# cshizhe/VLN-HAMT

Measured on AMD Instinct MI355X. Metric: panorama-steps/sec, R2R proxy pretrain (36x768 views, 80-tok instr), higher is better.
Workload: dtype bf16; 1 GPU; R2R 6-proxy-task pretrain step (fwd+bwd+clip+AdamW, dropout 0.1), fixed ViT features, R2R-canon model 174.8M params; per_gpu_batch=64, global_batch=64, txt_len=80, hist_len=5, views=36, task_mix=mlm:sap:sar:sprel:mrc:itm=5:1:1:1:2:2, parallelism=dp1, launch=hipGraph replay, dead_code_elimination=True

## Files before the change

### include/hamt.h

```cpp
#ifndef HAMT_H
#define HAMT_H

#include <stddef.h>
#include <stdint.h>

#ifdef __cplusplus
extern "C" {
#endif

#define HAMT_ABI_VERSION 2

typedef enum { HAMT_OK = 0, HAMT_ERR_ARG = -1, HAMT_ERR_UNSUPPORTED = -2, HAMT_ERR_LAUNCH = -3 } hamt_status;
typedef enum { HAMT_F32 = 0, HAMT_BF16 = 1,
               HAMT_U8G = 2,
               HAMT_F16 = 3 } hamt_dtype;
typedef enum { HAMT_PREC_BF16 = 0, HAMT_PREC_F32 = 1 } hamt_prec;

int hamt_version(void);
int hamt_last_error(char* buf, size_t n);
int hamt_last_kernel(char* buf, size_t n);
enum { HAMT_WS_GEMM_SPLITK = 0, HAMT_WS_COLSUM = 1, HAMT_WS_SUMSQ = 2, HAMT_WS_LN_BWD = 3, HAMT_WS_WGRAD_TABLE = 4, HAMT_WS_LNRED_TABLE = 5, HAMT_WS_VIS_EMBED_BWD = 6,
       HAMT_WS_EMBED_BWD = 7 ,
       HAMT_WS_OBJ_EMBED_BWD = 8, HAMT_WS_IMAGE_PREP = 9  };
size_t hamt_workspace_bytes(int op, const int* shape, int nshape);
// ... 37 lines not shown
  const void* dy;
  const void* x;
  float* dw;
  float* db;
  int M, N, K, ldy, ldx, ldw;
  int accum_dw, accum_db;
  float* ss;
  int K_valid;
  float wire_scale;
  const void* dy2;
  const void* x2;
  int K2, ldy2, ldx2, K2_valid;
} hamt_wgrad_desc;
#define HAMT_WGRAD_TABLE_ENTRY 112
int hamt_wgrad_grouped(int n, const hamt_wgrad_desc* probs, void* table, size_t table_bytes, void* stream);
int hamt_wgrad_grouped_ex(int n, const hamt_wgrad_desc* probs, void* table, size_t table_bytes, int phase, void* stream);

int hamt_colsum(int M, int N, const void* x, int ldx, int dtype_x, float* out, int accumulate,
                float* ws, void* stream);

typedef struct {
  int B, heads, Sq, Sk, d_head;
  int ldq, ldk, ldv, ldo;
  int dtype_qkv, dtype_o;
  float scale, p_drop;
  uint32_t call_id;
  int prec;
} hamt_attn_desc;
int hamt_attn_small_fwd(const hamt_attn_desc* d, const void* q, const void* k, const void* v,
                        const float* add_mask, void* o, float* lse, const uint64_t* rng, void* stream);
int hamt_attn_small_bwd(const hamt_attn_desc* d, const void* q, const void* k, const void* v,
                        const float* add_mask, const void* o, const void* d_o, const float* lse,
                        float* delta, void* dq, void* dk, void* dv, const uint64_t* rng, void* stream);

int hamt_attn_cls_fwd(const hamt_attn_desc* d, const void* q, const void* k, const void* v, void* o, void* stream);

int hamt_attn_varlen_fwd(const hamt_attn_desc* d, const void* q, const void* k, const void* v, const int* cu_seqlens,
                         void* o, float* lse, const uint64_t* rng, void* stream);
int hamt_attn_varlen_bwd(const hamt_attn_desc* d, const void* q, const void* k, const void* v, const int* cu_seqlens,
                         const void* o, const void* d_o, const float* lse, void* dq, void* dk, void* dv,
                         const uint64_t* rng, void* stream);
int hamt_attn_varlen_cross_fwd(const hamt_attn_desc* d, const void* q, const void* k, const void* v, const int* cu_q,
                               const int* cu_k, int n_pairs, const int* pair, const float* add_mask, void* o, float* lse,
                               const uint64_t* rng, void* stream);
int hamt_attn_varlen_cross_bwd(const hamt_attn_desc* d, const void* q, const void* k, const void* v, const int* cu_q,
                               const int* cu_k, int n_pairs, const int* pair, const float* add_mask, const void* o, const void* d_o,
                               const float* lse, void* dq, void* dk, void* dv, const uint64_t* rng, void* stream);

typedef struct {
  int M, H;
  int A;
  int ld_ang;
  float eps1, eps2;
  int x_bf16;
  int Mpad16;
} hamt_vis_embed_desc;
int hamt_vis_embed_fwd(const hamt_vis_embed_desc* d, const void* x1, const float* ang, const float* w_ang, const float* b_ang,
                       const float* gamma_img, const float* beta_img, const float* gamma_ang, const float* beta_ang,
                       float* y, void* y16, float* stats, void* stream);
int hamt_vis_embed_bwd(const hamt_vis_embed_desc* d, const float* dy, const void* x1, const float* ang, const float* w_ang,
                       const float* b_ang, const float* gamma_img, const float* gamma_ang, const float* stats, float* dx, void* dx16,
                       float* dgamma_img, float* dbeta_img, float* dgamma_ang, float* dbeta_ang, float* db_ang, float* dw_ang,
                       float* ws, void* stream);

typedef struct {
  int M, H;
// ... 280 lines not shown
```

### vln_hamt_amd/_lib.py

```python
from __future__ import annotations

import ctypes as C
import os

_HERE = os.path.dirname(os.path.abspath(__file__))
LIB_PATH = os.path.join(_HERE, "libhamt_hip.so")

HAMT_F32, HAMT_BF16, HAMT_U8G, HAMT_F16 = 0, 1, 2, 3
PREC_BF16, PREC_F32 = 0, 1
EPI_BIAS, EPI_GELU, EPI_RELU, EPI_ACCUM, EPI_MUL_DGELU, EPI_MUL_DRELU, EPI_SAVE_PRE = 1, 2, 4, 8, 16, 32, 64
EPI_GELU_GRAD, EPI_MUL_AUX, EPI_ADD_AUX, EPI_DROPOUT = 128, 256, 512, 1024
SUMSQ_SPARSE = 2
OPT_ADAMW, OPT_ADAM, OPT_RMSPROP, OPT_SGD = 0, 1, 2, 3

vp, i32, u32, f32, sz = C.c_void_p, C.c_int, C.c_uint32, C.c_float, C.c_size_t


class GemmDesc(C.Structure):
    _fields_ = [("M", i32), ("N", i32), ("K", i32), ("lda", i32), ("ldb", i32), ("ldc", i32), ("ldaux", i32),
                ("a_kmajor", i32), ("b_kmajor", i32), ("dtype_a", i32), ("dtype_b", i32), ("dtype_c", i32),
                ("dtype_aux", i32), ("prec", i32), ("epilogue", i32), ("alpha", f32), ("ka_rows", i32), ("kb_rows", i32),
                ("p_drop", f32), ("call_id", u32), ("rng", C.c_void_p)]


# ... 56 lines not shown


class ImageResampleDesc(C.Structure):
    _fields_ = [(n, i32) for n in ("n", "H", "W", "OH", "OW", "x0", "y0", "w", "h", "filter", "kx", "ky")]


WGRAD_TABLE_ENTRY = 112


class WgradDesc(C.Structure):
    _fields_ = [("dy", vp), ("x", vp), ("dw", vp), ("db", vp), ("M", i32), ("N", i32), ("K", i32), ("ldy", i32),
                ("ldx", i32), ("ldw", i32), ("accum_dw", i32), ("accum_db", i32), ("ss", vp), ("K_valid", i32),
                ("wire_scale", f32), ("dy2", vp), ("x2", vp), ("K2", i32), ("ldy2", i32), ("ldx2", i32), ("K2_valid", i32)]


SIGNATURES = {
    "hamt_version": [],
    "hamt_last_error": [C.c_char_p, sz],
    "hamt_last_kernel": [C.c_char_p, sz],
    "hamt_workspace_bytes": [i32, C.POINTER(i32), i32],
    "hamt_gemm": [C.POINTER(GemmDesc), vp, vp, vp, vp, vp, vp],
    "hamt_gemm_ksplit": [C.POINTER(GemmDesc)],
    "hamt_gemm_ws": [C.POINTER(GemmDesc), vp, vp, vp, vp, vp, vp, sz, vp],
    "hamt_gemm_plan": [C.POINTER(GemmDesc), sz, C.c_char_p, sz],
    "hamt_cast_pad_bf16": [i32, i32, i32, i32, vp, i32, vp, i32, vp],
    "hamt_cast_pad_bf16_dropout": [i32, i32, i32, vp, i32, vp, i32, f32, u32, vp, vp],
    "hamt_cast_transpose": [i32, i32, vp, i32, i32, vp, i32, i32, vp],
    "hamt_wgrad_grouped": [i32, C.POINTER(WgradDesc), vp, sz, vp],
    "hamt_wgrad_grouped_ex": [i32, C.POINTER(WgradDesc), vp, sz, i32, vp],
    "hamt_smallk_wgrad": [i32, i32, i32, vp, i32, vp, i32, vp, i32, vp, vp],
    "hamt_colsum": [i32, i32, vp, i32, i32, vp, i32, vp, vp],
    "hamt_attn_small_fwd": [C.POINTER(AttnDesc), vp, vp, vp, vp, vp, vp, vp, vp],
    "hamt_attn_small_bwd": [C.POINTER(AttnDesc), vp, vp, vp, vp, vp, vp, vp, vp, vp, vp, vp, vp, vp],
    "hamt_attn_cls_fwd": [C.POINTER(AttnDesc), vp, vp, vp, vp, vp],
    "hamt_attn_varlen_fwd": [C.POINTER(AttnDesc), vp, vp, vp, vp, vp, vp, vp, vp],
    "hamt_attn_varlen_bwd": [C.POINTER(AttnDesc), vp, vp, vp, vp, vp, vp, vp, vp, vp, vp, vp, vp],
    "hamt_attn_varlen_cross_fwd": [C.POINTER(AttnDesc), vp, vp, vp, vp, vp, C.c_int, vp, vp, vp, vp, vp, vp],
    "hamt_attn_varlen_cross_bwd": [C.POINTER(AttnDesc), vp, vp, vp, vp, vp, C.c_int, vp, vp, vp, vp, vp, vp, vp, vp, vp, vp],
    "hamt_vis_embed_fwd": [C.POINTER(VisEmbedDesc)] + [vp] * 12,
    "hamt_vis_embed_bwd": [C.POINTER(VisEmbedDesc)] + [vp] * 18,
    "hamt_obj_embed_fwd": [C.POINTER(ObjEmbedDesc), C.POINTER(ObjEmbedParams)] + [vp] * 7,
    "hamt_obj_embed_bwd": [C.POINTER(ObjEmbedDesc), C.POINTER(ObjEmbedParams), C.POINTER(ObjEmbedGrads)] + [vp] * 10,
    "hamt_ln_fwd": [C.POINTER(LnDesc), vp, vp, vp, vp, vp, vp, vp, vp, vp, vp, vp],
    "hamt_ln_bwd": [C.POINTER(LnDesc), vp, vp, vp, vp, vp, vp, vp, vp, vp, vp, vp, vp, vp, vp],
    "hamt_ln_bwd_add": [C.POINTER(LnDesc), vp, vp, vp, vp, vp, vp, vp, vp, vp, vp, vp],
    "hamt_ln_bwd_reduce": [i32, i32, vp, vp, vp, vp, vp],
    "hamt_ln_bwd_reduce_grouped": [i32, vp, vp, sz, vp],
    "hamt_gather_rows": [i32, i32, vp, i32, vp, vp, i32, vp, i32, i32, vp],
    "hamt_scatter_add_rows": [i32, i32, vp, i32, i32, vp, vp, i32, vp],
    "hamt_scatter_add_rows_small": [i32, i32, vp, i32, i32, vp, i32, vp, vp, vp],
    "hamt_scatter_add_rows_ordered": [i32, i32, vp, i32, i32, vp, vp, i32, i32, vp, vp],
    "hamt_embed_sum_fwd": [i32, i32, i32, vp, vp, vp, vp, vp, vp],
    "hamt_embed_sum_bwd": [i32, i32, i32, i32, vp, vp, vp, vp, vp, vp, sz, vp],
    "hamt_mean_mid_fwd": [i32, i32, i32, vp, vp, vp],
    "hamt_mean_mid_bwd": [i32, i32, i32, vp, vp, vp],
    "hamt_mul_bcast_fwd": [i32, i32, i32, vp, vp, i32, vp, vp],
    "hamt_mul_bcast_bwd": [i32, i32, i32, vp, vp, i32, vp, vp, vp, vp],
    "hamt_sum_rows": [i32, i32, i32, vp, i32, vp, vp, vp],
    "hamt_patchify": [i32, i32, i32, i32, i32, vp, vp, i32, i32, i32, vp],
    "hamt_image_prep": [C.POINTER(ImagePrepDesc), vp, vp, vp, vp, vp, vp, sz, vp],
    "hamt_image_resample_taps": [i32, i32, i32, i32, i32, vp, vp, vp, i32],
    "hamt_image_resample": [C.POINTER(ImageResampleDesc), vp, vp, vp, vp, vp, vp, vp],
    "hamt_add3": [sz, vp, vp, vp, vp, vp],
    "hamt_dropout": [sz, vp, vp, f32, u32, vp, vp],
    "hamt_cast_f32_bf16": [sz, vp, vp, vp],
    "hamt_unpack_padded": [vp, vp, i32, i32, i32, i32, vp, vp],
# ... 65 lines not shown
        raise HamtError(f"{LIB_PATH} is missing: build it with `python vln_hamt_amd/csrc/build.py` "
                        "(there is no CPU/PyTorch fallback for the HAMT kernels)")
    import torch
    lib = C.CDLL(LIB_PATH)
    for name, args in SIGNATURES.items():
        fn = getattr(lib, name)
        fn.argtypes = args
        fn.restype = sz if name == "hamt_workspace_bytes" else i32
    if lib.hamt_version() != 2:
        raise HamtError("libhamt_hip.so ABI version mismatch")
    _lib = lib
    return lib


def last_error() -> str:
    buf = C.create_string_buffer(512)
    load().hamt_last_error(buf, 512)
    return buf.value.decode(errors="replace")


def last_kernel() -> str:
    buf = C.create_string_buffer(160)
    load().hamt_last_kernel(buf, 160)
    return buf.value.decode(errors="replace")


def gemm_plan(desc: GemmDesc, ws_bytes=None):
    buf = C.create_string_buffer(160)
    ks = load().hamt_gemm_plan(C.byref(desc), sz(-1).value if ws_bytes is None else ws_bytes, buf, 160)
    check(min(ks, 0), "hamt_gemm_plan")
    return ks, buf.value.decode(errors="replace")


def workspace_bytes(op: int, *shape) -> int:
    arr = (i32 * max(1, len(shape)))(*shape)
    return int(load().hamt_workspace_bytes(op, arr, len(shape)))


WS_GEMM_SPLITK, WS_COLSUM, WS_SUMSQ, WS_LN_BWD, WS_WGRAD_TABLE, WS_LNRED_TABLE, WS_VIS_EMBED_BWD, WS_EMBED_BWD, WS_OBJ_EMBED_BWD = range(9)
WS_IMAGE_PREP = 9


def check(rc: int, name: str):
    if rc != 0:
        raise HamtError(f"{name} failed (status {rc}): {last_error()}")
```

### vln_hamt_amd/csrc/attn16.hip

```cpp
#include "common.h"

namespace {

constexpr int T64 = 64;
constexpr int AST = 72;
typedef __attribute__((address_space(3))) s16x4 lds_s16x4;

struct Attn16Args {
  hamt_attn_desc d;
  const void *q, *k, *v, *o, *d_o;
  const float* mask;
  void *out, *dq, *dk, *dv;
  float* lse;
  const uint64_t* rng;
  const int* cu_q;
  const int* cu_k;
  int n_pairs;
  const int* pair;
};

template <typename T> __device__ __forceinline__ void ld8(const T* p, float (&f)[8]);
template <> __device__ __forceinline__ void ld8<float>(const float* p, float (&f)[8]) {
  const float4 a = ((const float4*)p)[0], b = ((const float4*)p)[1];
  f[0] = a.x; f[1] = a.y; f[2] = a.z; f[3] = a.w; f[4] = b.x; f[5] = b.y; f[6] = b.z; f[7] = b.w;
}
template <> __device__ __forceinline__ void ld8<bf16_t>(const bf16_t* p, float (&f)[8]) {
  const uint4 x = *(const uint4*)p;
  const uint32_t u[4] = {x.x, x.y, x.z, x.w};
#pragma unroll
  for (int j = 0; j < 4; ++j) { f[2 * j] = __uint_as_float(u[j] << 16); f[2 * j + 1] = __uint_as_float(u[j] & 0xffff0000u); }
}
__device__ __forceinline__ uint4 pack8(const float (&f)[8]) {
  return make_uint4(pack_bf2(f[0], f[1]), pack_bf2(f[2], f[3]), pack_bf2(f[4], f[5]), pack_bf2(f[6], f[7]));
}
template <typename T> __device__ __forceinline__ void st4(T* p, float a, float b, float c, float d);
template <> __device__ __forceinline__ void st4<float>(float* p, float a, float b, float c, float d) { *(float4*)p = make_float4(a, b, c, d); }
template <> __device__ __forceinline__ void st4<bf16_t>(bf16_t* p, float a, float b, float c, float d) { *(uint2*)p = make_uint2(pack_bf2(a, b), pack_bf2(c, d)); }
template <typename T> __device__ __forceinline__ float4 ld4(const T* p);
// ... 419 lines not shown
  float rs = 0.f;
  f32x4 of[4];
#pragma unroll
  for (int i = 0; i < 4; ++i) of[i] = (f32x4){0.f, 0.f, 0.f, 0.f};
#pragma unroll
  for (int s = 0; s < KB / 2; ++s) {
    float p[2][4];
#pragma unroll
    for (int e = 0; e < 2; ++e) {
#pragma unroll
      for (int r = 0; r < 4; ++r) { p[e][r] = __expf(sf[2 * s + e][r] - mn); rs += p[e][r]; }
      if (d.p_drop > 0.f) {
        float ds4[4];
        drop_scale4(key, rowh, (uint32_t)(4 * (2 * s + e) + g), d.p_drop, inv_keep, ds4);
#pragma unroll
        for (int r = 0; r < 4; ++r) p[e][r] *= ds4[r];
      }
    }
    const bf16x8 pf = pack_frag(p[0], p[1]);
#pragma unroll
    for (int db = 0; db < 4; ++db) of[db] = MFMA16(tfrag(Vs, 32 * s + 4 * g, 32 * s + 16 + 4 * g, 16 * db, lane), pf, of[db]);
  }
  const float l_run = xg_sum(rs);
  if (qok) {
    TO* O = (TO*)a.out + qrow0 * d.ldo + h * 64 + (size_t)qrow * d.ldo;
    const float inv = 1.0f / l_run;
#pragma unroll
    for (int db = 0; db < 4; ++db) st4<TO>(O + 16 * db + 4 * g, of[db][0] * inv, of[db][1] * inv, of[db][2] * inv, of[db][3] * inv);
    if (g == 0) a.lse[((size_t)b * d.heads + h) * d.Sq + qrow] = mn + __logf(l_run);
  }
}

template <typename TI, typename TO, int NB>
__global__ __launch_bounds__(512) void attn_s128_bwd_kernel(Attn16Args a) {
  extern __shared__ __attribute__((aligned(16))) bf16_t sm[];
  const hamt_attn_desc& d = a.d;
  const int t = threadIdx.x, nt = blockDim.x, lane = t & 63, w = t >> 6, l15 = lane & 15, g = lane >> 4;
  const int h = blockIdx.x, b = blockIdx.y;
  int Sq = d.Sq, Sk = d.Sk;
  size_t qrow0 = (size_t)b * d.Sq, krow0 = (size_t)b * d.Sk;
  if (a.cu_q) { const int c0 = a.cu_q[b]; Sq = a.cu_q[b + 1] - c0; qrow0 = (size_t)c0; }
  if (Sq <= 0) return;
  const int kb_ = a.pair ? a.pair[b] : b;
  const bool filler = a.pair ? kb_ < 0 : ((a.cu_q || a.cu_k) && b >= a.n_pairs);
  if (!filler) {
    krow0 = (size_t)kb_ * d.Sk;
    if (a.cu_k) { const int c0 = a.cu_k[kb_]; Sk = a.cu_k[kb_ + 1] - c0; krow0 = (size_t)c0; }
  }
  if (filler || Sk <= 0) {
    TI* dQ0 = (TI*)a.dq + qrow0 * d.ldq + h * 64;
    for (int i = t; i < Sq * 8; i += nt) { st4<TI>(dQ0 + (size_t)(i >> 3) * d.ldq + (i & 7) * 8, 0.f, 0.f, 0.f, 0.f); st4<TI>(dQ0 + (size_t)(i >> 3) * d.ldq + (i & 7) * 8 + 4, 0.f, 0.f, 0.f, 0.f); }
    return;
  }
  const int nqb = (Sq + 15) >> 4, nkb = (Sk + 15) >> 4, sq16 = nqb * 16, sk16 = nkb * 16, PST = sq16 + 8;
  bf16_t* Qs = sm;
  bf16_t* dOs = Qs + sq16 * AST;
  bf16_t* Ks = dOs + sq16 * AST;
  bf16_t* Vs = Ks + sk16 * AST;
  bf16_t* Pt = Vs + sk16 * AST;
  bf16_t* dSt = Pt + sk16 * PST;
  float* lse_s = (float*)(dSt + sk16 * PST);
  float* delta_s = lse_s + sq16;
  float* mk_s = delta_s + sq16;
  const TI* Q = (const TI*)a.q + qrow0 * d.ldq + h * 64;
  const TI* K = (const TI*)a.k + krow0 * d.ldk + h * 64;
  const TI* V = (const TI*)a.v + krow0 * d.ldv + h * 64;
  const TO* O = (const TO*)a.o + qrow0 * d.ldo + h * 64;
  const TO* dO = (const TO*)a.d_o + qrow0 * d.ldo + h * 64;
  {
    Raw8<TI> rq[2], rk[2], rv[2];
    Raw8<TO> rdo[2], ro[2];
    rows_load<TI, 2>(Q, d.ldq, Sq, t, nt, rq);
    rows_load<TO, 2>(dO, d.ldo, Sq, t, nt, rdo);
    rows_load<TO, 2>(O, d.ldo, Sq, t, nt, ro);
    rows_load<TI, 2>(K, d.ldk, Sk, t, nt, rk);
    rows_load<TI, 2>(V, d.ldv, Sk, t, nt, rv);
    stage_mask(a.cu_k ? nullptr : a.mask, kb_, Sk, sk16, mk_s, t, nt);
    for (int i = t; i < sk16 * PST / 8; i += nt) { ((uint4*)Pt)[i] = make_uint4(0, 0, 0, 0); ((uint4*)dSt)[i] = make_uint4(0, 0, 0, 0); }
    rows_store<TI, 2>(rq, sq16, Qs, t, nt);
    rows_store<TO, 2>(rdo, sq16, dOs, t, nt);
#pragma unroll
    for (int i = 0; i < 2; ++i) {
      const int r = (t >> 3) + i * (nt >> 3);
      float f[8], o8[8], acc = 0.f;
      raw_f32(rdo[i], f);
      raw_f32(ro[i], o8);
#pragma unroll
      for (int j = 0; j < 8; ++j) acc += f[j] * o8[j];
      acc += __shfl_xor(acc, 1, 64); acc += __shfl_xor(acc, 2, 64); acc += __shfl_xor(acc, 4, 64);
      if ((t & 7) == 0 && r < sq16) { delta_s[r] = acc; lse_s[r] = r < Sq ? a.lse[((size_t)b * d.heads + h) * d.Sq + r] : 0.f; }
    }
    rows_store<TI, 2>(rk, sk16, Ks, t, nt);
    rows_store<TI, 2>(rv, sk16, Vs, t, nt);
  }
  __syncthreads();
  const RngKey key = rng_key(a.rng, d.call_id);
  const float inv_keep = d.p_drop > 0.f ? 1.0f / (1.0f - d.p_drop) : 1.0f;
  if (w < nqb) {
    const int ql = 16 * w + l15;
    bf16x8 qf[2], df[2];
#pragma unroll
    for (int s = 0; s < 2; ++s) { qf[s] = rfrag(Qs, ql, 32 * s + 8 * g); df[s] = rfrag(dOs, ql, 32 * s + 8 * g); }
    const float lse_q = lse_s[ql], delta_q = delta_s[ql];
    const uint32_t rowh = hamt_mix32((uint32_t)((b * d.heads + h) * d.Sq + ql) ^ key.k0);
    const bool qv = ql < Sq;
#pragma unroll
    for (int kb = 0; kb < NB; ++kb) {
      if (kb < nkb) {
        f32x4 sf = (f32x4){0.f, 0.f, 0.f, 0.f}, dpf = (f32x4){0.f, 0.f, 0.f, 0.f};
#pragma unroll
        for (int s = 0; s < 2; ++s) {
          sf = MFMA16(rfrag(Ks, 16 * kb + l15, 32 * s + 8 * g), qf[s], sf);
          dpf = MFMA16(rfrag(Vs, 16 * kb + l15, 32 * s + 8 * g), df[s], dpf);
        }
        const float4 mk = *(const float4*)(mk_s + 16 * kb + 4 * g);
        const float mk4[4] = {mk.x, mk.y, mk.z, mk.w};
        float ds4[4] = {1.f, 1.f, 1.f, 1.f};
        if (d.p_drop > 0.f) drop_scale4(key, rowh, (uint32_t)(4 * kb + g), d.p_drop, inv_keep, ds4);
#pragma unroll
        for (int r = 0; r < 4; ++r) {
          const int kk = 16 * kb + 4 * g + r;
          const float pr = __expf(fmaf(sf[r], d.scale, mk4[r]) - lse_q);
          if (qv) {
            Pt[kk * PST + ql] = f2bf(pr * ds4[r]);
            dSt[kk * PST + ql] = f2bf(pr * (dpf[r] * ds4[r] - delta_q) * d.scale);
          }
        }
      }
    }
  }
  __syncthreads();
  if (w < nkb) {
    f32x4 dkf[4], dvf[4];
#pragma unroll
    for (int i = 0; i < 4; ++i) { dkf[i] = (f32x4){0.f, 0.f, 0.f, 0.f}; dvf[i] = (f32x4){0.f, 0.f, 0.f, 0.f}; }
#pragma unroll
    for (int s = 0; s < NB / 2; ++s) {
      if (2 * s < nqb) {
        const bf16x8 pb = rfrag_lim(Pt, PST, 16 * w + l15, 32 * s + 8 * g, sq16), sb = rfrag_lim(dSt, PST, 16 * w + l15, 32 * s + 8 * g, sq16);
#pragma unroll
        for (int db = 0; db < 4; ++db) {
          dvf[db] = MFMA16(tfrag_lim(dOs, AST, 32 * s + 8 * g, 32 * s + 8 * g + 4, sq16, 16 * db, lane), pb, dvf[db]);
          dkf[db] = MFMA16(tfrag_lim(Qs, AST, 32 * s + 8 * g, 32 * s + 8 * g + 4, sq16, 16 * db, lane), sb, dkf[db]);
        }
      }
    }
    const int kk = 16 * w + l15;
    if (kk < Sk) {
      TI* dK = (TI*)a.dk + krow0 * d.ldk + h * 64 + (size_t)kk * d.ldk;
      TI* dV = (TI*)a.dv + krow0 * d.ldv + h * 64 + (size_t)kk * d.ldv;
#pragma unroll
      for (int db = 0; db < 4; ++db) {
        st4<TI>(dK + 16 * db + 4 * g, dkf[db][0], dkf[db][1], dkf[db][2], dkf[db][3]);
        st4<TI>(dV + 16 * db + 4 * g, dvf[db][0], dvf[db][1], dvf[db][2], dvf[db][3]);
      }
    }
  }
  if (w < nqb) {
    f32x4 dqf[4];
#pragma unroll
    for (int i = 0; i < 4; ++i) dqf[i] = (f32x4){0.f, 0.f, 0.f, 0.f};
#pragma unroll
    for (int s = 0; s < NB / 2; ++s) {
      if (2 * s < nkb) {
        const bf16x8 sb = tfrag_lim(dSt, PST, 32 * s + 8 * g, 32 * s + 8 * g + 4, sk16, 16 * w, lane);
#pragma unroll
        for (int db = 0; db < 4; ++db) dqf[db] = MFMA16(tfrag_lim(Ks, AST, 32 * s + 8 * g, 32 * s + 8 * g + 4, sk16, 16 * db, lane), sb, dqf[db]);
      }
    }
    const int qq = 16 * w + l15;
    if (qq < Sq) {
      TI* dQ = (TI*)a.dq + qrow0 * d.ldq + h * 64 + (size_t)qq * d.ldq;
#pragma unroll
      for (int db = 0; db < 4; ++db) st4<TI>(dQ + 16 * db + 4 * g, dqf[db][0], dqf[db][1], dqf[db][2], dqf[db][3]);
    }
  }
}

template <typename TI, typename TO, bool PACKED>
__global__ __launch_bounds__(1024) void attn_wide_bwd_kernel(Attn16Args a) {
  extern __shared__ __attribute__((aligned(16))) bf16_t sm[];
  const hamt_attn_desc& d = a.d;
  const int t = threadIdx.x, nt = blockDim.x, lane = t & 63, w = t >> 6, l15 = lane & 15, g = lane >> 4;
  const int h = blockIdx.x, b = blockIdx.y;
  int Sq = d.Sq, Sk = d.Sk;
  size_t qrow0 = (size_t)b * d.Sq, krow0 = (size_t)b * d.Sk;
  const float* mask = a.mask;
  int mrow = b;
  if constexpr (PACKED) {
    if (a.cu_q) { const int c0 = a.cu_q[b]; Sq = a.cu_q[b + 1] - c0; qrow0 = (size_t)c0; }
    if (Sq <= 0) return;
    mrow = a.pair ? a.pair[b] : b;
    const bool filler = a.pair ? mrow < 0 : b >= a.n_pairs;
    if (!filler) {
      krow0 = (size_t)mrow * d.Sk;
      if (a.cu_k) { const int c0 = a.cu_k[mrow]; Sk = a.cu_k[mrow + 1] - c0; krow0 = (size_t)c0; mask = nullptr; }
    }
    if (filler || Sk <= 0) {
      TI* dQ0 = (TI*)a.dq + qrow0 * d.ldq + h * 64;
      for (int i = t; i < Sq * 16; i += nt) st4<TI>(dQ0 + (size_t)(i >> 4) * d.ldq + (i & 15) * 4, 0.f, 0.f, 0.f, 0.f);
      return;
    }
  }
  const int nqb = (Sq + 15) >> 4, nkb = (Sk + 15) >> 4, sq16 = nqb * 16, sk16 = nkb * 16;
  bf16_t* Qs = sm;
// ... 119 lines not shown
          for (int r = 0; r < 4; ++r) {
            const float pr = __expf(fmaf(sf[r], d.scale, mk) - lq[r]);
            float keep = 1.f;
            if (d.p_drop > 0.f) {
              uint32_t x = hamt_mix32(rh[r] + grp_h);
              if (second) x = hamt_mix32(x ^ 0x85ebca6bu);
              keep = (high ? (x >> 16) : (x & 0xffffu)) >= thr ? inv_keep : 0.0f;
            }
            const bool qv = 16 * qb + 4 * g + r < Sq;
            pt[e][r] = qv ? pr * keep : 0.f;
            dsv[e][r] = qv ? pr * (dpf[r] * keep - dq_[r]) * d.scale : 0.f;
          }
        }
      }
      const bf16x8 pb = pack_frag(pt[0], pt[1]), sb = pack_frag(dsv[0], dsv[1]);
#pragma unroll
      for (int db = 0; db < 4; ++db) {
        dvf[db] = MFMA16(tfrag_lim(dOs, AST, 32 * s + 4 * g, 32 * s + 16 + 4 * g, sq16, 16 * db, lane), pb, dvf[db]);
        dkf[db] = MFMA16(tfrag_lim(Qs, AST, 32 * s + 4 * g, 32 * s + 16 + 4 * g, sq16, 16 * db, lane), sb, dkf[db]);
      }
    }
    if (kl < Sk) {
      TI* dK = (TI*)a.dk + krow0 * d.ldk + h * 64 + (size_t)kl * d.ldk;
      TI* dV = (TI*)a.dv + krow0 * d.ldv + h * 64 + (size_t)kl * d.ldv;
#pragma unroll
      for (int db = 0; db < 4; ++db) {
        st4<TI>(dK + 16 * db + 4 * g, dkf[db][0], dkf[db][1], dkf[db][2], dkf[db][3]);
        st4<TI>(dV + 16 * db + 4 * g, dvf[db][0], dvf[db][1], dvf[db][2], dvf[db][3]);
      }
    }
  }
}

size_t wide_bwd_lds(const hamt_attn_desc& d) {
  const int sq16 = (d.Sq + 15) / 16 * 16, sk16 = (d.Sk + 15) / 16 * 16;
  return (size_t)2 * (sq16 + sk16) * AST * sizeof(bf16_t) + (size_t)(3 * sq16 + sk16) * sizeof(float);
}

template <typename TI, typename TO, bool PACKED>
void launch_wide_bwd(const Attn16Args& a, hipStream_t s) {
  const hamt_attn_desc& d = a.d;
  const int nqb = (d.Sq + 15) / 16, nkb = (d.Sk + 15) / 16, nb = nqb > nkb ? nqb : nkb;
  static bool raised = false;
  if (!raised) {
    (void)hipFuncSetAttribute(reinterpret_cast<const void*>(&attn_wide_bwd_kernel<TI, TO, PACKED>), hipFuncAttributeMaxDynamicSharedMemorySize, 160 * 1024);
    raised = true;
  }
  hipLaunchKernelGGL((attn_wide_bwd_kernel<TI, TO, PACKED>), dim3(d.heads, d.B), dim3(64 * nb), wide_bwd_lds(d), s, a);
}

template <typename TI, typename TO, int KB, int IT>
void launch_s128_fwd_kb(const Attn16Args& a, dim3 grid, dim3 block, size_t lds, hipStream_t s) {
  static bool raised = false;
  if (lds > 64 * 1024 && !raised) {
    hipFuncSetAttribute(reinterpret_cast<const void*>(&attn_s128_fwd_kernel<TI, TO, KB, IT>), hipFuncAttributeMaxDynamicSharedMemorySize, 160 * 1024);
    raised = true;
  }
  hipLaunchKernelGGL((attn_s128_fwd_kernel<TI, TO, KB, IT>), grid, block, lds, s, a);
}

template <typename TI, typename TO>
void launch_s128_fwd(const Attn16Args& a, hipStream_t s) {
  const hamt_attn_desc& d = a.d;
  const int nqb = (d.Sq + 15) / 16, nkb = (d.Sk + 15) / 16;
  const int kb = nkb <= 2 ? 2 : (nkb + 1) & ~1;
  const int it = kb > 8 ? 4 : 2;
  const int need = 2 * kb / it;
  const int nqw = nqb < 8 ? nqb : 8;
  const int nw = nqw > need ? nqw : need;
  const dim3 grid(d.heads, d.B, (d.Sq + 127) / 128), block(64 * nw);
  const size_t lds = (size_t)2 * kb * 16 * AST * sizeof(bf16_t) + (size_t)kb * 16 * sizeof(float);
  switch (kb) {
    case 2: launch_s128_fwd_kb<TI, TO, 2, 2>(a, grid, block, lds, s); break;
    case 4: launch_s128_fwd_kb<TI, TO, 4, 2>(a, grid, block, lds, s); break;
    case 6: launch_s128_fwd_kb<TI, TO, 6, 2>(a, grid, block, lds, s); break;
    case 8: launch_s128_fwd_kb<TI, TO, 8, 2>(a, grid, block, lds, s); break;
    case 10: launch_s128_fwd_kb<TI, TO, 10, 4>(a, grid, block, lds, s); break;
    case 12: launch_s128_fwd_kb<TI, TO, 12, 4>(a, grid, block, lds, s); break;
    case 14: launch_s128_fwd_kb<TI, TO, 14, 4>(a, grid, block, lds, s); break;
    default: launch_s128_fwd_kb<TI, TO, 16, 4>(a, grid, block, lds, s); break;
  }
}

template <typename TI, typename TO, int NB>
void launch_s128_bwd_nb(const Attn16Args& a, dim3 grid, dim3 block, size_t lds, hipStream_t s) {
  static bool raised = false;
  if (!raised) {
    hipFuncSetAttribute(reinterpret_cast<const void*>(&attn_s128_bwd_kernel<TI, TO, NB>), hipFuncAttributeMaxDynamicSharedMemorySize, 160 * 1024);
    raised = true;
  }
  hipLaunchKernelGGL((attn_s128_bwd_kernel<TI, TO, NB>), grid, block, lds, s, a);
}

template <typename TI, typename TO>
void launch_s128_bwd(const Attn16Args& a, hipStream_t s) {
  const hamt_attn_desc& d = a.d;
  const int nqb = (d.Sq + 15) / 16, nkb = (d.Sk + 15) / 16, nb = nqb > nkb ? nqb : nkb;
  const int sq16 = nqb * 16, sk16 = nkb * 16;
  const dim3 grid(d.heads, d.B), block(64 * nb);
  const size_t lds = ((size_t)2 * (sq16 + sk16) * AST + (size_t)2 * sk16 * (sq16 + 8)) * sizeof(bf16_t) + (size_t)(2 * sq16 + sk16) * sizeof(float);
  if (nb <= 2) launch_s128_bwd_nb<TI, TO, 2>(a, grid, block, lds, s);
  else if (nb <= 4) launch_s128_bwd_nb<TI, TO, 4>(a, grid, block, lds, s);
  else if (nb <= 6) launch_s128_bwd_nb<TI, TO, 6>(a, grid, block, lds, s);
  else launch_s128_bwd_nb<TI, TO, 8>(a, grid, block, lds, s);
}

bool use_s128_fwd(const hamt_attn_desc* d) {
  static const bool off = getenv("HAMT_NO_ATTN_S128") != nullptr;
  static const bool off_wide = getenv("HAMT_NO_ATTN_WIDE") != nullptr;
  return !off && d->Sk <= (off_wide ? 128 : 256) && (d->Sq <= 128 || !off_wide);
}
bool use_s128_bwd(const hamt_attn_desc* d) {
  static const bool off = getenv("HAMT_NO_ATTN_S128") != nullptr;
  return !off && d->Sq <= 128 && d->Sk <= 128;
}
bool use_wide_bwd(const hamt_attn_desc* d) {
  static const bool off = getenv("HAMT_NO_ATTN_WIDE_BWD") != nullptr;
  return !off && d->Sq <= 224 && d->Sk <= 224;
}

}

void hamt_attn16_fwd_launch(const hamt_attn_desc* d, const void* q, const void* k, const void* v, const float* mask, void* o,
                            float* lse, const uint64_t* rng, hipStream_t s, const int* cu_q, const int* cu_k, int n_pairs, const int* pair) {
  Attn16Args a{*d, q, k, v, nullptr, nullptr, mask, o, nullptr, nullptr, nullptr, lse, rng, cu_q, cu_k, n_pairs, pair};
  const int* cu = cu_q ? cu_q : cu_k;
  dim3 grid((d->Sq + T64 - 1) / T64, d->heads, d->B), block(256);
  const bool ib = d->dtype_qkv == HAMT_BF16, ob = d->dtype_o == HAMT_BF16;
  if (use_s128_fwd(d) || cu) {
    if (!ib && !ob) launch_s128_fwd<float, float>(a, s);
    else if (ib && ob) launch_s128_fwd<bf16_t, bf16_t>(a, s);
    else if (ib) launch_s128_fwd<bf16_t, float>(a, s);
    else launch_s128_fwd<float, bf16_t>(a, s);
    return;
  }
  if (!ib && !ob) hipLaunchKernelGGL((attn16_fwd_kernel<float, float>), grid, block, 0, s, a);
  else if (ib && ob) hipLaunchKernelGGL((attn16_fwd_kernel<bf16_t, bf16_t>), grid, block, 0, s, a);
  else if (ib) hipLaunchKernelGGL((attn16_fwd_kernel<bf16_t, float>), grid, block, 0, s, a);
  else hipLaunchKernelGGL((attn16_fwd_kernel<float, bf16_t>), grid, block, 0, s, a);
}

void hamt_attn16_bwd_launch(const hamt_attn_desc* d, const void* q, const void* k, const void* v, const float* mask, const void* o,
                            const void* d_o, const float* lse, void* dq, void* dk, void* dv, const uint64_t* rng, hipStream_t s,
                            const int* cu_q, const int* cu_k, int n_pairs, const int* pair) {
  Attn16Args a{*d, q, k, v, o, d_o, mask, nullptr, dq, dk, dv, const_cast<float*>(lse), rng, cu_q, cu_k, n_pairs, pair};
  const int* cu = cu_q ? cu_q : cu_k;
  dim3 grid(d->heads, d->B), block(256);
  const bool ib = d->dtype_qkv == HAMT_BF16, ob = d->dtype_o == HAMT_BF16;
  if (cu && (d->Sq > 128 || d->Sk > 128)) {
    hamt_set_last_kernel("attn_wide_bwd_kernel<packed>");
    if (!ib && !ob) launch_wide_bwd<float, float, true>(a, s);
    else if (ib && ob) launch_wide_bwd<bf16_t, bf16_t, true>(a, s);
    else if (ib) launch_wide_bwd<bf16_t, float, true>(a, s);
    else launch_wide_bwd<float, bf16_t, true>(a, s);
    return;
  }
  if (use_s128_bwd(d) || cu) {
    hamt_set_last_kernel("attn_s128_bwd_kernel");
    if (!ib && !ob) launch_s128_bwd<float, float>(a, s);
    else if (ib && ob) launch_s128_bwd<bf16_t, bf16_t>(a, s);
    else if (ib) launch_s128_bwd<bf16_t, float>(a, s);
    else launch_s128_bwd<float, bf16_t>(a, s);
    return;
  }
  if (use_wide_bwd(d)) {
    hamt_set_last_kernel("attn_wide_bwd_kernel");
    if (!ib && !ob) launch_wide_bwd<float, float, false>(a, s);
    else if (ib && ob) launch_wide_bwd<bf16_t, bf16_t, false>(a, s);
    else if (ib) launch_wide_bwd<bf16_t, float, false>(a, s);
    else launch_wide_bwd<float, bf16_t, false>(a, s);
    return;
  }
  hamt_set_last_kernel("attn16_bwd_kernel");
  if (!ib && !ob) hipLaunchKernelGGL((attn16_bwd_kernel<float, float>), grid, block, 0, s, a);
  else if (ib && ob) hipLaunchKernelGGL((attn16_bwd_kernel<bf16_t, bf16_t>), grid, block, 0, s, a);
  else if (ib) hipLaunchKernelGGL((attn16_bwd_kernel<bf16_t, float>), grid, block, 0, s, a);
  else hipLaunchKernelGGL((attn16_bwd_kernel<float, bf16_t>), grid, block, 0, s, a);
}
```

Measured before the change: 6517 panorama-steps/s.

## Reuse one LDS buffer for P and dS in s128 attention backward

The s128 attention backward kernel now keeps P and dS in registers and stages them one at a time through a single LDS buffer that aliases the V tile. dV is computed and stored first, then dS overwrites the same buffer for dK and dQ. The zero-fill of the two P/dS buffers is removed and launch bounds now request more resident blocks for small NB. The goal is a much smaller LDS footprint so more workgroups fit per CU. The cost is extra __syncthreads barriers and more registers per thread. A plan helper and a debug occupancy query API are also added.

Result: no change. 6556 panorama-steps/s, median of 6 (+0.6%).

```diff
diff --git a/include/hamt.h b/include/hamt.h
--- a/include/hamt.h
+++ b/include/hamt.h
@@ -93,6 +93,8 @@
 int hamt_attn_small_bwd(const hamt_attn_desc* d, const void* q, const void* k, const void* v,
                         const float* add_mask, const void* o, const void* d_o, const float* lse,
                         float* delta, void* dq, void* dk, void* dv, const uint64_t* rng, void* stream);
+int hamt_attn_bwd_plan(const hamt_attn_desc* d, int packed, int* lds_bytes, int* threads, char* name, size_t n);
+int hamt_debug_attn_bwd_resident(const hamt_attn_desc* d);
 
 int hamt_attn_cls_fwd(const hamt_attn_desc* d, const void* q, const void* k, const void* v, void* o, void* stream);
 
diff --git a/vln_hamt_amd/_lib.py b/vln_hamt_amd/_lib.py
--- a/vln_hamt_amd/_lib.py
+++ b/vln_hamt_amd/_lib.py
@@ -112,6 +112,8 @@
     "hamt_colsum": [i32, i32, vp, i32, i32, vp, i32, vp, vp],
     "hamt_attn_small_fwd": [C.POINTER(AttnDesc), vp, vp, vp, vp, vp, vp, vp, vp],
     "hamt_attn_small_bwd": [C.POINTER(AttnDesc), vp, vp, vp, vp, vp, vp, vp, vp, vp, vp, vp, vp, vp],
+    "hamt_attn_bwd_plan": [C.POINTER(AttnDesc), i32, C.POINTER(i32), C.POINTER(i32), C.c_char_p, sz],
+    "hamt_debug_attn_bwd_resident": [C.POINTER(AttnDesc)],
     "hamt_attn_cls_fwd": [C.POINTER(AttnDesc), vp, vp, vp, vp, vp],
     "hamt_attn_varlen_fwd": [C.POINTER(AttnDesc), vp, vp, vp, vp, vp, vp, vp, vp],
     "hamt_attn_varlen_bwd": [C.POINTER(AttnDesc), vp, vp, vp, vp, vp, vp, vp, vp, vp, vp, vp, vp],
@@ -243,6 +245,13 @@
     return ks, buf.value.decode(errors="replace")
 
 
+def attn_bwd_plan(desc: AttnDesc, packed=False):
+    buf, lds, threads = C.create_string_buffer(64), i32(0), i32(0)
+    n = load().hamt_attn_bwd_plan(C.byref(desc), int(packed), C.byref(lds), C.byref(threads), buf, 64)
+    check(min(n, 0), "hamt_attn_bwd_plan")
+    return n, lds.value, threads.value, buf.value.decode(errors="replace")
+
+
 def workspace_bytes(op: int, *shape) -> int:
     arr = (i32 * max(1, len(shape)))(*shape)
     return int(load().hamt_workspace_bytes(op, arr, len(shape)))
diff --git a/vln_hamt_amd/csrc/attn16.hip b/vln_hamt_amd/csrc/attn16.hip
--- a/vln_hamt_amd/csrc/attn16.hip
+++ b/vln_hamt_amd/csrc/attn16.hip
@@ -1,9 +1,10 @@
 #include "common.h"
+#include "attn_plan.h"
 
 namespace {
 
 constexpr int T64 = 64;
-constexpr int AST = 72;
+constexpr int AST = ATTN_AST;
 typedef __attribute__((address_space(3))) s16x4 lds_s16x4;
 
 struct Attn16Args {
@@ -489,7 +490,7 @@
 }
 
 template <typename TI, typename TO, int NB>
-__global__ __launch_bounds__(512) void attn_s128_bwd_kernel(Attn16Args a) {
+__global__ __launch_bounds__(64 * NB, NB <= 6 ? 5 : 2) void attn_s128_bwd_kernel(Attn16Args a) {
   extern __shared__ __attribute__((aligned(16))) bf16_t sm[];
   const hamt_attn_desc& d = a.d;
   const int t = threadIdx.x, nt = blockDim.x, lane = t & 63, w = t >> 6, l15 = lane & 15, g = lane >> 4;
@@ -514,9 +515,8 @@
   bf16_t* dOs = Qs + sq16 * AST;
   bf16_t* Ks = dOs + sq16 * AST;
   bf16_t* Vs = Ks + sk16 * AST;
-  bf16_t* Pt = Vs + sk16 * AST;
-  bf16_t* dSt = Pt + sk16 * PST;
-  float* lse_s = (float*)(dSt + sk16 * PST);
+  bf16_t* Bt = Vs;
+  float* lse_s = (float*)(Vs + sk16 * (PST > AST ? PST : AST));
   float* delta_s = lse_s + sq16;
   float* mk_s = delta_s + sq16;
   const TI* Q = (const TI*)a.q + qrow0 * d.ldq + h * 64;
@@ -533,7 +533,6 @@
     rows_load<TI, 2>(K, d.ldk, Sk, t, nt, rk);
     rows_load<TI, 2>(V, d.ldv, Sk, t, nt, rv);
     stage_mask(a.cu_k ? nullptr : a.mask, kb_, Sk, sk16, mk_s, t, nt);
-    for (int i = t; i < sk16 * PST / 8; i += nt) { ((uint4*)Pt)[i] = make_uint4(0, 0, 0, 0); ((uint4*)dSt)[i] = make_uint4(0, 0, 0, 0); }
     rows_store<TI, 2>(rq, sq16, Qs, t, nt);
     rows_store<TO, 2>(rdo, sq16, dOs, t, nt);
 #pragma unroll
@@ -553,8 +552,9 @@
   __syncthreads();
   const RngKey key = rng_key(a.rng, d.call_id);
   const float inv_keep = d.p_drop > 0.f ? 1.0f / (1.0f - d.p_drop) : 1.0f;
+  const int ql = 16 * w + l15;
+  uint2 pp[NB], sp[NB];
   if (w < nqb) {
-    const int ql = 16 * w + l15;
     bf16x8 qf[2], df[2];
 #pragma unroll
     for (int s = 0; s < 2; ++s) { qf[s] = rfrag(Qs, ql, 32 * s + 8 * g); df[s] = rfrag(dOs, ql, 32 * s + 8 * g); }
@@ -574,43 +574,75 @@
         const float mk4[4] = {mk.x, mk.y, mk.z, mk.w};
         float ds4[4] = {1.f, 1.f, 1.f, 1.f};
         if (d.p_drop > 0.f) drop_scale4(key, rowh, (uint32_t)(4 * kb + g), d.p_drop, inv_keep, ds4);
+        float pv[4], sv[4];
 #pragma unroll
         for (int r = 0; r < 4; ++r) {
-          const int kk = 16 * kb + 4 * g + r;
           const float pr = __expf(fmaf(sf[r], d.scale, mk4[r]) - lse_q);
-          if (qv) {
-            Pt[kk * PST + ql] = f2bf(pr * ds4[r]);
-            dSt[kk * PST + ql] = f2bf(pr * (dpf[r] * ds4[r] - delta_q) * d.scale);
-          }
-        }
+          pv[r] = pr * ds4[r];
+          sv[r] = pr * (dpf[r] * ds4[r] - delta_q) * d.scale;
+        }
+        pp[kb] = qv ? make_uint2(pack_bf2(pv[0], pv[1]), pack_bf2(pv[2], pv[3])) : make_uint2(0, 0);
+        sp[kb] = qv ? make_uint2(pack_bf2(sv[0], sv[1]), pack_bf2(sv[2], sv[3])) : make_uint2(0, 0);
+      }
+    }
+  }
+  __syncthreads();
+  if (w < nqb) {
+#pragma unroll
+    for (int kb = 0; kb < NB; ++kb) {
+      if (kb < nkb) {
+        bf16_t* col = Bt + (16 * kb + 4 * g) * PST + ql;
+        col[0] = (bf16_t)pp[kb].x; col[PST] = (bf16_t)(pp[kb].x >> 16); col[2 * PST] = (bf16_t)pp[kb].y; col[3 * PST] = (bf16_t)(pp[kb].y >> 16);
+      }
+    }
+  }
+  __syncthreads();
+  const int kk = 16 * w + l15;
+  if (w < nkb) {
+    f32x4 dvf[4];
+#pragma unroll
+    for (int i = 0; i < 4; ++i) dvf[i] = (f32x4){0.f, 0.f, 0.f, 0.f};
+#pragma unroll
+    for (int s = 0; s < NB / 2; ++s) {
+      if (2 * s < nqb) {
+        const bf16x8 pb = rfrag_lim(Bt, PST, kk, 32 * s + 8 * g, sq16);
+#pragma unroll
+        for (int db = 0; db < 4; ++db) dvf[db] = MFMA16(tfrag_lim(dOs, AST, 32 * s + 8 * g, 32 * s + 8 * g + 4, sq16, 16 * db, lane), pb, dvf[db]);
+      }
+    }
+    if (kk < Sk) {
+      TI* dV = (TI*)a.dv + krow0 * d.ldv + h * 64 + (size_t)kk * d.ldv;
+#pragma unroll
+      for (int db = 0; db < 4; ++db) st4<TI>(dV + 16 * db + 4 * g, dvf[db][0], dvf[db][1], dvf[db][2], dvf[db][3]);
+    }
+  }
+  __syncthreads();
+  if (w < nqb) {
+#pragma unroll
+    for (int kb = 0; kb < NB; ++kb) {
+      if (kb < nkb) {
+        bf16_t* col = Bt + (16 * kb + 4 * g) * PST + ql;
+        col[0] = (bf16_t)sp[kb].x; col[PST] = (bf16_t)(sp[kb].x >> 16); col[2 * PST] = (bf16_t)sp[kb].y; col[3 * PST] = (bf16_t)(sp[kb].y >> 16);
       }
     }
   }
   __syncthreads();
   if (w < nkb) {
-    f32x4 dkf[4], dvf[4];
-#pragma unroll
-    for (int i = 0; i < 4; ++i) { dkf[i] = (f32x4){0.f, 0.f, 0.f, 0.f}; dvf[i] = (f32x4){0.f, 0.f, 0.f, 0.f}; }
+    f32x4 dkf[4];
+#pragma unroll
+    for (int i = 0; i < 4; ++i) dkf[i] = (f32x4){0.f, 0.f, 0.f, 0.f};
 #pragma unroll
     for (int s = 0; s < NB / 2; ++s) {
       if (2 * s < nqb) {
-        const bf16x8 pb = rfrag_lim(Pt, PST, 16 * w + l15, 32 * s + 8 * g, sq16), sb = rfrag_lim(dSt, PST, 16 * w + l15, 32 * s + 8 * g, sq16);
-#pragma unroll
-        for (int db = 0; db < 4; ++db) {
-          dvf[db] = MFMA16(tfrag_lim(dOs, AST, 32 * s + 8 * g, 32 * s + 8 * g + 4, sq16, 16 * db, lane), pb, dvf[db]);
-          dkf[db] = MFMA16(tfrag_lim(Qs, AST, 32 * s + 8 * g, 32 * s + 8 * g + 4, sq16, 16 * db, lane), sb, dkf[db]);
-        }
-      }
-    }
-    const int kk = 16 * w + l15;
+        const bf16x8 sb = rfrag_lim(Bt, PST, kk, 32 * s + 8 * g, sq16);
+#pragma unroll
+        for (int db = 0; db < 4; ++db) dkf[db] = MFMA16(tfrag_lim(Qs, AST, 32 * s + 8 * g, 32 * s + 8 * g + 4, sq16, 16 * db, lane), sb, dkf[db]);
+      }
+    }
     if (kk < Sk) {
       TI* dK = (TI*)a.dk + krow0 * d.ldk + h * 64 + (size_t)kk * d.ldk;
-      TI* dV = (TI*)a.dv + krow0 * d.ldv + h * 64 + (size_t)kk * d.ldv;
-#pragma unroll
-      for (int db = 0; db < 4; ++db) {
-        st4<TI>(dK + 16 * db + 4 * g, dkf[db][0], dkf[db][1], dkf[db][2], dkf[db][3]);
-        st4<TI>(dV + 16 * db + 4 * g, dvf[db][0], dvf[db][1], dvf[db][2], dvf[db][3]);
-      }
+#pragma unroll
+      for (int db = 0; db < 4; ++db) st4<TI>(dK + 16 * db + 4 * g, dkf[db][0], dkf[db][1], dkf[db][2], dkf[db][3]);
     }
   }
   if (w < nqb) {
@@ -620,14 +652,13 @@
 #pragma unroll
     for (int s = 0; s < NB / 2; ++s) {
       if (2 * s < nkb) {
-        const bf16x8 sb = tfrag_lim(dSt, PST, 32 * s + 8 * g, 32 * s + 8 * g + 4, sk16, 16 * w, lane);
+        const bf16x8 sb = tfrag_lim(Bt, PST, 32 * s + 8 * g, 32 * s + 8 * g + 4, sk16, 16 * w, lane);
 #pragma unroll
         for (int db = 0; db < 4; ++db) dqf[db] = MFMA16(tfrag_lim(Ks, AST, 32 * s + 8 * g, 32 * s + 8 * g + 4, sk16, 16 * db, lane), sb, dqf[db]);
       }
     }
-    const int qq = 16 * w + l15;
-    if (qq < Sq) {
-      TI* dQ = (TI*)a.dq + qrow0 * d.ldq + h * 64 + (size_t)qq * d.ldq;
+    if (ql < Sq) {
+      TI* dQ = (TI*)a.dq + qrow0 * d.ldq + h * 64 + (size_t)ql * d.ldq;
 #pragma unroll
       for (int db = 0; db < 4; ++db) st4<TI>(dQ + 16 * db + 4 * g, dqf[db][0], dqf[db][1], dqf[db][2], dqf[db][3]);
     }
@@ -813,21 +844,15 @@
   }
 }
 
-size_t wide_bwd_lds(const hamt_attn_desc& d) {
-  const int sq16 = (d.Sq + 15) / 16 * 16, sk16 = (d.Sk + 15) / 16 * 16;
-  return (size_t)2 * (sq16 + sk16) * AST * sizeof(bf16_t) + (size_t)(3 * sq16 + sk16) * sizeof(float);
-}
-
 template <typename TI, typename TO, bool PACKED>
-void launch_wide_bwd(const Attn16Args& a, hipStream_t s) {
+void launch_wide_bwd(const Attn16Args& a, const AttnBwdPlan& p, hipStream_t s) {
   const hamt_attn_desc& d = a.d;
-  const int nqb = (d.Sq + 15) / 16, nkb = (d.Sk + 15) / 16, nb = nqb > nkb ? nqb : nkb;
   static bool raised = false;
   if (!raised) {
     (void)hipFuncSetAttribute(reinterpret_cast<const void*>(&attn_wide_bwd_kernel<TI, TO, PACKED>), hipFuncAttributeMaxDynamicSharedMemorySize, 160 * 1024);
     raised = true;
   }
-  hipLaunchKernelGGL((attn_wide_bwd_kernel<TI, TO, PACKED>), dim3(d.heads, d.B), dim3(64 * nb), wide_bwd_lds(d), s, a);
+  hipLaunchKernelGGL((attn_wide_bwd_kernel<TI, TO, PACKED>), dim3(d.heads, d.B), dim3(p.threads), p.lds, s, a);
 }
 
 template <typename TI, typename TO, int KB, int IT>
@@ -864,26 +889,36 @@
 }
 
 template <typename TI, typename TO, int NB>
-void launch_s128_bwd_nb(const Attn16Args& a, dim3 grid, dim3 block, size_t lds, hipStream_t s) {
+int s128_bwd_nb(const Attn16Args& a, const AttnBwdPlan& p, hipStream_t s, bool launch) {
   static bool raised = false;
   if (!raised) {
     hipFuncSetAttribute(reinterpret_cast<const void*>(&attn_s128_bwd_kernel<TI, TO, NB>), hipFuncAttributeMaxDynamicSharedMemorySize, 160 * 1024);
     raised = true;
   }
-  hipLaunchKernelGGL((attn_s128_bwd_kernel<TI, TO, NB>), grid, block, lds, s, a);
+  if (launch) {
+    hipLaunchKernelGGL((attn_s128_bwd_kernel<TI, TO, NB>), dim3(a.d.heads, a.d.B), dim3(p.threads), p.lds, s, a);
+    return 0;
+  }
+  int n = 0;
+  const hipError_t e = hipOccupancyMaxActiveBlocksPerMultiprocessor(&n, reinterpret_cast<const void*>(&attn_s128_bwd_kernel<TI, TO, NB>), p.threads, p.lds);
+  return e == hipSuccess ? n : -1;
 }
 
 template <typename TI, typename TO>
-void launch_s128_bwd(const Attn16Args& a, hipStream_t s) {
-  const hamt_attn_desc& d = a.d;
-  const int nqb = (d.Sq + 15) / 16, nkb = (d.Sk + 15) / 16, nb = nqb > nkb ? nqb : nkb;
-  const int sq16 = nqb * 16, sk16 = nkb * 16;
-  const dim3 grid(d.heads, d.B), block(64 * nb);
-  const size_t lds = ((size_t)2 * (sq16 + sk16) * AST + (size_t)2 * sk16 * (sq16 + 8)) * sizeof(bf16_t) + (size_t)(2 * sq16 + sk16) * sizeof(float);
-  if (nb <= 2) launch_s128_bwd_nb<TI, TO, 2>(a, grid, block, lds, s);
-  else if (nb <= 4) launch_s128_bwd_nb<TI, TO, 4>(a, grid, block, lds, s);
-  else if (nb <= 6) launch_s128_bwd_nb<TI, TO, 6>(a, grid, block, lds, s);
-  else launch_s128_bwd_nb<TI, TO, 8>(a, grid, block, lds, s);
+int s128_bwd(const Attn16Args& a, const AttnBwdPlan& p, hipStream_t s, bool launch) {
+  switch (p.nb) {
+    case 2: return s128_bwd_nb<TI, TO, 2>(a, p, s, launch);
+    case 4: return s128_bwd_nb<TI, TO, 4>(a, p, s, launch);
+    case 6: return s128_bwd_nb<TI, TO, 6>(a, p, s, launch);
+    default: return s128_bwd_nb<TI, TO, 8>(a, p, s, launch);
+  }
+}
+int s128_bwd_typed(const Attn16Args& a, const AttnBwdPlan& p, hipStream_t s, bool launch) {
+  const bool ib = a.d.dtype_qkv == HAMT_BF16, ob = a.d.dtype_o == HAMT_BF16;
+  if (!ib && !ob) return s128_bwd<float, float>(a, p, s, launch);
+  if (ib && ob) return s128_bwd<bf16_t, bf16_t>(a, p, s, launch);
+  if (ib) return s128_bwd<bf16_t, float>(a, p, s, launch);
+  return s128_bwd<float, bf16_t>(a, p, s, launch);
 }
 
 bool use_s128_fwd(const hamt_attn_desc* d) {
@@ -891,13 +926,9 @@
   static const bool off_wide = getenv("HAMT_NO_ATTN_WIDE") != nullptr;
   return !off && d->Sk <= (off_wide ? 128 : 256) && (d->Sq <= 128 || !off_wide);
 }
-bool use_s128_bwd(const hamt_attn_desc* d) {
-  static const bool off = getenv("HAMT_NO_ATTN_S128") != nullptr;
-  return !off && d->Sq <= 128 && d->Sk <= 128;
-}
-bool use_wide_bwd(const hamt_attn_desc* d) {
-  static const bool off = getenv("HAMT_NO_ATTN_WIDE_BWD") != nullptr;
-  return !off && d->Sq <= 224 && d->Sk <= 224;
+const AttnBwdSwitches& bwd_switches() {
+  static const AttnBwdSwitches sw{getenv("HAMT_NO_ATTN_S128") != nullptr, getenv("HAMT_NO_ATTN_WIDE_BWD") != nullptr};
+  return sw;
 }
 
 }
@@ -928,33 +959,57 @@
   const int* cu = cu_q ? cu_q : cu_k;
   dim3 grid(d->heads, d->B), block(256);
   const bool ib = d->dtype_qkv == HAMT_BF16, ob = d->dtype_o == HAMT_BF16;
-  if (cu && (d->Sq > 128 || d->Sk > 128)) {
-    hamt_set_last_kernel("attn_wide_bwd_kernel<packed>");
-    if (!ib && !ob) launch_wide_bwd<float, float, true>(a, s);
-    else if (ib && ob) launch_wide_bwd<bf16_t, bf16_t, true>(a, s);
-    else if (ib) launch_wide_bwd<bf16_t, float, true>(a, s);
-    else launch_wide_bwd<float, bf16_t, true>(a, s);
+  const AttnBwdPlan pl = attn_bwd_plan(*d, cu != nullptr, bwd_switches());
+  char name[40];
+  attn_bwd_plan_name(pl, name, sizeof(name));
+  hamt_set_last_kernel("%s", name);
+  if (pl.family == ATTN_BWD_WIDE_PACKED) {
+    if (!ib && !ob) launch_wide_bwd<float, float, true>(a, pl, s);
+    else if (ib && ob) launch_wide_bwd<bf16_t, bf16_t, true>(a, pl, s);
+    else if (ib) launch_wide_bwd<bf16_t, float, true>(a, pl, s);
+    else launch_wide_bwd<float, bf16_t, true>(a, pl, s);
     return;
   }
-  if (use_s128_bwd(d) || cu) {
-    hamt_set_last_kernel("attn_s128_bwd_kernel");
-    if (!ib && !ob) launch_s128_bwd<float, float>(a, s);
-    else if (ib && ob) launch_s128_bwd<bf16_t, bf16_t>(a, s);
-    else if (ib) launch_s128_bwd<bf16_t, float>(a, s);
-    else launch_s128_bwd<float, bf16_t>(a, s);
+  if (pl.family == ATTN_BWD_S128) {
+    s128_bwd_typed(a, pl, s, true);
     return;
   }
-  if (use_wide_bwd(d)) {
-    hamt_set_last_kernel("attn_wide_bwd_kernel");
-    if (!ib && !ob) launch_wide_bwd<float, float, false>(a, s);
-    else if (ib && ob) launch_wide_bwd<bf16_t, bf16_t, false>(a, s);
-    else if (ib) launch_wide_bwd<bf16_t, float, false>(a, s);
-    else launch_wide_bwd<float, bf16_t, false>(a, s);
+  if (pl.family == ATTN_BWD_WIDE) {
+    if (!ib && !ob) launch_wide_bwd<float, float, false>(a, pl, s);
+    else if (ib && ob) launch_wide_bwd<bf16_t, bf16_t, false>(a, pl, s);
+    else if (ib) launch_wide_bwd<bf16_t, float, false>(a, pl, s);
+    else launch_wide_bwd<float, bf16_t, false>(a, pl, s);
     return;
   }
-  hamt_set_last_kernel("attn16_bwd_kernel");
   if (!ib && !ob) hipLaunchKernelGGL((attn16_bwd_kernel<float, float>), grid, block, 0, s, a);
   else if (ib && ob) hipLaunchKernelGGL((attn16_bwd_kernel<bf16_t, bf16_t>), grid, block, 0, s, a);
   else if (ib) hipLaunchKernelGGL((attn16_bwd_kernel<bf16_t, float>), grid, block, 0, s, a);
   else hipLaunchKernelGGL((attn16_bwd_kernel<float, bf16_t>), grid, block, 0, s, a);
 }
+
+extern "C" int hamt_attn_bwd_plan(const hamt_attn_desc* d, int packed, int* lds_bytes, int* threads, char* name, size_t n) {
+  HAMT_CHECK_ARG(d && (name || n == 0), "hamt_attn_bwd_plan: null pointer");
+  HAMT_CHECK_ARG(d->heads > 0 && d->Sq > 0 && d->Sk > 0 && (!packed || (d->Sq <= 256 && d->Sk <= 256)), "hamt_attn_bwd_plan: bad sizes (Sq %d, Sk %d)", d->Sq, d->Sk);
+  const AttnBwdPlan p = attn_bwd_plan(*d, packed != 0, bwd_switches());
+  if (lds_bytes) *lds_bytes = (int)p.lds;
+  if (threads) *threads = p.threads;
+  if (n) attn_bwd_plan_name(p, name, n);
+  return p.resident;
+}
+
+extern "C" int hamt_debug_attn_bwd_resident(const hamt_attn_desc* d) {
+  HAMT_CHECK_ARG(d && d->heads > 0 && d->Sq > 0 && d->Sk > 0, "hamt_debug_attn_bwd_resident: bad descriptor");
+  const AttnBwdPlan p = attn_bwd_plan(*d, false, bwd_switches());
+  if (p.family != ATTN_BWD_S128) {
+    hamt_set_error("hamt_debug_attn_bwd_resident: %d x %d does not run on attn_s128_bwd_kernel", d->Sq, d->Sk);
+    return HAMT_ERR_UNSUPPORTED;
+  }
+  Attn16Args a{};
+  a.d = *d;
+  const int r = s128_bwd_typed(a, p, nullptr, false);
+  if (r < 0) {
+    hamt_set_error("hamt_debug_attn_bwd_resident: the occupancy query failed: %s", hipGetErrorString(hipGetLastError()));
+    return HAMT_ERR_LAUNCH;
+  }
+  return r;
+}
diff --git a/vln_hamt_amd/csrc/attn_plan.h b/vln_hamt_amd/csrc/attn_plan.h
--- /dev/null
+++ b/vln_hamt_amd/csrc/attn_plan.h
@@ -0,0 +1,52 @@
+#pragma once
+#include "../../include/hamt.h"
+#include <stddef.h>
+#include <stdio.h>
+
+constexpr int ATTN_AST = 72;
+constexpr int ATTN_CU_LDS = 160 * 1024;
+constexpr int ATTN_CU_WAVES = 32;
+
+struct AttnBwdSwitches {
+  bool no_s128;
+  bool no_wide_bwd;
+};
+
+enum AttnBwdFamily { ATTN_BWD_S128, ATTN_BWD_WIDE, ATTN_BWD_WIDE_PACKED, ATTN_BWD_TILED, ATTN_BWD_F32 };
+
+struct AttnBwdPlan {
+  AttnBwdFamily family;
+  int nb;
+  int threads;
+  size_t lds;
+  int resident;
+};
+
+static inline size_t attn_s128_bwd_lds(int Sq, int Sk) {
+  const int sq16 = (Sq + 15) / 16 * 16, sk16 = (Sk + 15) / 16 * 16, pst = sq16 + 8;
+  return ((size_t)(2 * sq16 + sk16) * ATTN_AST + (size_t)sk16 * (pst > ATTN_AST ? pst : ATTN_AST)) * 2 + (size_t)(2 * sq16 + sk16) * sizeof(float);
+}
+static inline size_t attn_wide_bwd_lds(int Sq, int Sk) {
+  const int sq16 = (Sq + 15) / 16 * 16, sk16 = (Sk + 15) / 16 * 16;
+  return (size_t)2 * (sq16 + sk16) * ATTN_AST * 2 + (size_t)(3 * sq16 + sk16) * sizeof(float);
+}
+
+static inline AttnBwdPlan attn_bwd_plan(const hamt_attn_desc& d, bool packed, const AttnBwdSwitches& sw) {
+  AttnBwdPlan p{ATTN_BWD_TILED, 0, 256, 0, 0};
+  if (d.prec != HAMT_PREC_BF16) { p.family = ATTN_BWD_F32; return p; }
+  const int nqb = (d.Sq + 15) / 16, nkb = (d.Sk + 15) / 16, nb = nqb > nkb ? nqb : nkb;
+  const bool small = d.Sq <= 128 && d.Sk <= 128;
+  if (packed && !small) { p.family = ATTN_BWD_WIDE_PACKED; p.nb = nb; p.lds = attn_wide_bwd_lds(d.Sq, d.Sk); }
+  else if (packed || (small && !sw.no_s128)) { p.family = ATTN_BWD_S128; p.nb = nb <= 2 ? 2 : nb <= 4 ? 4 : nb <= 6 ? 6 : 8; p.lds = attn_s128_bwd_lds(d.Sq, d.Sk); }
+  else if (!sw.no_wide_bwd && d.Sq <= 224 && d.Sk <= 224) { p.family = ATTN_BWD_WIDE; p.nb = nb; p.lds = attn_wide_bwd_lds(d.Sq, d.Sk); }
+  else return p;
+  p.threads = 64 * nb;
+  const int by_lds = (int)(ATTN_CU_LDS / p.lds), by_waves = ATTN_CU_WAVES / nb;
+  p.resident = by_lds < by_waves ? by_lds : by_waves;
+  return p;
+}
+
+static inline int attn_bwd_plan_name(const AttnBwdPlan& p, char* buf, size_t n) {
+  static const char* const names[] = {"attn_s128_bwd_kernel", "attn_wide_bwd_kernel", "attn_wide_bwd_kernel<packed>", "attn16_bwd_kernel", "attn_bwd_kernel"};
+  return snprintf(buf, n, "%s", names[p.family]);
+}
```
